# VinAIResearch/tise-toolbox

Measured on AMD Instinct MI355X. Metric: images/sec through InceptionV3+FID on 30k 256x256 @1/2/4/8 GPU; |dFID| vs ref, higher is better.
Workload: dtype f32 (split 2xf16 operands, 3 f16 MFMAs/product, f32 accumulate)

## Files before the change

tise_toolbox_amd/csrc/conv_pipe.hip:

```cpp
#include <stdlib.h>
#include <string.h>
#include <hip/hip_fp16.h>
#include "common.h"
#include "conv_epilogue.h"

namespace {

typedef _Float16 half8_t __attribute__((ext_vector_type(8)));
typedef _Float16 half4_t __attribute__((ext_vector_type(4)));
typedef float float16_t __attribute__((ext_vector_type(16)));
typedef float float4_t __attribute__((ext_vector_type(4)));
typedef unsigned int u32x4_t __attribute__((ext_vector_type(4)));
typedef tise_conv_args ConvArgs;
typedef __attribute__((address_space(3))) void* lds_ptr_t;

__device__ __attribute__((aligned(64))) unsigned char g_pipe_zero_page[64];

#define CP_BK 32

__device__ __forceinline__ bool wrap_guard(long long tile, long long ntiles) { return tile < ntiles; }

__device__ __forceinline__ int pool_swz(int slot) { return ((slot & 3) << 2) ^ ((slot >> 1) & 1); }
constexpr int POOL_HV_SLOTS = 130;

template <int COUT, bool PADDED, bool DBG = false, bool POOL = false>
__global__ __launch_bounds__(512, 2) void conv_regw32_kernel(const ConvArgs p, const int R16, const long long ntiles) {
    static_assert(!POOL || (COUT == 64 && !PADDED && !DBG), "pooled output: Conv2d_2b's instance only");
    constexpr int KHC = 3, KWC = 3, ntaps = 9;
    constexpr int TPI = 64 / COUT;
    constexpr int PF = COUT == 64 ? 2 : 1;
    constexpr int NPW = 2 * TPI;
    constexpr int STEP = 128 * TPI;
    constexpr int STG = conv_epi::Staging<1>::BYTES;
    extern __shared__ __attribute__((aligned(1024))) unsigned char lds[];
    const int tid = threadIdx.x, lane = tid & 63;
    const int wave = __builtin_amdgcn_readfirstlane(tid >> 6);
    const int ms = wave & 3, grp = wave >> 2;
    const int ring = R16 + STEP * PF;
    unsigned char* wbuf = lds;
    unsigned char* epi_area = wbuf + ring * 128;
    unsigned char* stage = epi_area + 2048 + wave * STG;
    unsigned char* vbuf = epi_area + 2048;
    unsigned char* hvbuf = vbuf + p.OW * 256;

    const long long G = (long long)gridDim.x;
    const long long mgrid = (long long)p.N * p.H * p.W;
    const int minoff = -p.PH * p.W - p.PW;
    const unsigned char* xg = reinterpret_cast<const unsigned char*>(p.x);
    const unsigned char* zp = g_pipe_zero_page;
    const long long niter_all = (ntiles + TPI - 1) / TPI;
    const long long per = (niter_all + G - 1) / G;
    const long long i_begin = (long long)blockIdx.x * per, i_end = (i_begin + per < niter_all) ? i_begin + per : niter_all;
    if (!POOL && i_begin >= niter_all) return;
    const int ohp = (p.OH - 3) / 2 + 1, owp = (p.OW - 3) / 2 + 1;
    long long g_start = 0;
    unsigned glen = 0;
    if (POOL) {
        const long long units = (long long)p.N * ohp;
        const long long u0 = units * blockIdx.x / G, u1 = units * (blockIdx.x + 1) / G;
        if (u0 >= u1) return;
        const long long n0 = u0 / ohp, n1 = (u1 - 1) / ohp;
        const int oy0 = (int)(u0 - n0 * ohp), oy1 = (int)(u1 - 1 - n1 * ohp);
        g_start = (n0 * p.H + 2 * oy0) * p.W;
        glen = (unsigned)((n1 * p.H + 2 * oy1 + 3) * p.W - g_start);
    }
    const long long t_begin = i_begin * TPI;
    const long long g_base = (POOL ? g_start : t_begin * 128) + minoff;
    const int nit = POOL ? (int)((glen + 127u) / 128u) : (int)(i_end - i_begin);

    half8_t bw[ntaps][2][2];
    {
        const _Float16* wgt = reinterpret_cast<const _Float16*>(p.w);
        const int cout = (COUT == 64 ? grp * 32 : 0) + (lane & 15);
        const _Float16* wrow = wgt + (long long)cout * p.Kpad + (lane >> 4) * 8;
#pragma unroll
        for (int t = 0; t < ntaps; ++t)
#pragma unroll
            for (int s2 = 0; s2 < 2; ++s2) {
                bw[t][s2][0] = *reinterpret_cast<const half8_t*>(wrow + (long long)s2 * 16 * p.Kpad + t * CP_BK);
                bw[t][s2][1] = *reinterpret_cast<const half8_t*>(wrow + (long long)s2 * 16 * p.Kpad + p.w_plane + t * CP_BK);
            }
#pragma unroll
        for (int t = 0; t < ntaps; ++t)
#pragma unroll
            for (int s2 = 0; s2 < 2; ++s2) {
                asm volatile("" : "+v"(bw[t][s2][0]));
                asm volatile("" : "+v"(bw[t][s2][1]));
            }
    }
#define RW32_ROWS(REL0, PROW0, NPIECES, Q0, QS)                                                           \
    {                                                                                                     \
        for (int q = (Q0); q < (NPIECES); q += (QS)) {                                                     \
            const long long g = g_base + (REL0) + q * 8 + (lane >> 3);                                     \
            const bool ok = g >= 0 && g < mgrid;                                                           \
            int prow = (PROW0) + q * 8;                                                                    \
            while (prow >= ring) prow -= ring;                                  \
            const int c = (lane & 7) ^ ((lane >> 4) << 1);     \
            const unsigned char* src = xg + g * 128 + c * 16;                                              \
            src = ok ? src : zp;                                                                           \
            __builtin_amdgcn_global_load_lds(src, (lds_ptr_t)(wbuf + prow * 128), 16, 0, 0);               \
        }                                                                                                  \
    }
    RW32_ROWS(0LL, 0, (R16 >> 3) + 16 * TPI * (PF - 1), wave, 8)
    {
        conv_epi::float4_t sc_pre = {0.f, 0.f, 0.f, 0.f}, bs_pre = {0.f, 0.f, 0.f, 0.f};
        if (tid < COUT / 4) {
            sc_pre = *reinterpret_cast<const conv_epi::float4_t*>(p.scale + 4 * tid);
            bs_pre = *reinterpret_cast<const conv_epi::float4_t*>(p.bias + 4 * tid);
        }
        static_assert(conv_epi::EpiArea<COUT>::BYTES <= 2048, "epilogue area");
        conv_epi::prepare<COUT>(p, epi_area, 0, sc_pre, bs_pre);
    }
    const unsigned W_ = (unsigned)p.W, H_ = (unsigned)p.H;
    const unsigned sx = (unsigned)STEP % W_, syf = (unsigned)STEP / W_;
    const unsigned sy = syf % H_, sn = syf / H_;
    unsigned en, ey, ex, cy[2] = {0, 0}, cx[2] = {0, 0};
    {
        const unsigned hw = H_ * W_;
        const unsigned g0 = (unsigned)(POOL ? g_start : t_begin * 128) + (TPI == 2 ? grp * 128 : 0) + ms * 32;
        const unsigned ge = g0 + (lane >> 3);
        en = ge / hw;
        const unsigned rem = ge - en * hw;
        ey = rem / W_; ex = rem - ey * W_;
        if (PADDED || POOL) {
#pragma unroll
            for (int pi = 0; pi < 2; ++pi) {
                const unsigned gc = g0 + pi * 16 + (lane & 15);
                const unsigned remc = gc % hw;
                cy[pi] = remc / W_; cx[pi] = remc - cy[pi] * W_;
            }
        }
    }
    unsigned tn_ = 0, ty_ = 0, tx_ = 0;
    if (POOL) {
        const unsigned hw = H_ * W_;
        tn_ = (unsigned)g_start / hw;
        ty_ = ((unsigned)g_start - tn_ * hw) / W_;
    }
    int toff[ntaps];
#pragma unroll
    for (int t = 0; t < ntaps; ++t) toff[t] = (t / KWC - p.PH) * p.W + (t % KWC - p.PW);
    const int lrow0 = (TPI == 2 ? grp * 128 : 0) + ms * 32 + (lane & 15) - minoff;
    const int l4 = lane >> 4;
    const unsigned ringB = (unsigned)ring * 128u;
    unsigned a0t[ntaps];
#pragma unroll
    for (int t = 0; t < ntaps; ++t) {
        int wrow = lrow0 + toff[t];
        wrow = wrow >= ring ? wrow - ring : wrow;
        a0t[t] = (unsigned)(wrow * 128 + ((l4 ^ tise_lds_swz(wrow)) << 4));
    }
    asm volatile("s_waitcnt vmcnt(0)" ::: "memory");
    __syncthreads();

    conv_epi::Acc16 acc_main[1][1], acc_corr[1][1];
    int wstart = 0;
    int pnew = (R16 + (PF - 1) * STEP) % ring;
    long long relnew = (long long)R16 + (PF - 1) * STEP;
    for (int it = 0; it < nit; ++it) {
        const bool ahead = it + PF < nit;
        if (ahead && !(DBG && (p.nseg & 0x100))) { RW32_ROWS(relnew, pnew, 16 * TPI, wave, 8) }
        const long long tile = t_begin + (long long)it * TPI + (TPI == 2 ? grp : 0);
        unsigned tapmask[2] = {0x1ffu, 0x1ffu};
        if (PADDED) {
#pragma unroll
            for (int pi = 0; pi < 2; ++pi) {
                tapmask[pi] = 0u;
#pragma unroll
                for (int t = 0; t < ntaps; ++t) {
                    const int yy = (int)cy[pi] + t / KWC - p.PH, xx = (int)cx[pi] + t % KWC - p.PW;
                    if (yy >= 0 && yy < p.H && xx >= 0 && xx < p.W) tapmask[pi] |= 1u << t;
                }
            }
        }
        half8_t fa_[2][2][2];
#define RW32_READS(TAP, BUF)                                                                              \
        {                                                                                                  \
            const unsigned a0 = a0t[TAP];                                                                  \
            const unsigned a1u = a0 + 2048u - ringB;           \
            const unsigned a1 = a1u < a1u + ringB ? a1u : a1u + ringB;                                     \
            u32x4_t ah0 = *reinterpret_cast<const u32x4_t*>(wbuf + a0);                                    \
            u32x4_t al0 = *reinterpret_cast<const u32x4_t*>(wbuf + (a0 ^ 64));                             \
            u32x4_t ah1 = *reinterpret_cast<const u32x4_t*>(wbuf + a1);                                    \
            u32x4_t al1 = *reinterpret_cast<const u32x4_t*>(wbuf + (a1 ^ 64));                             \
            if (PADDED) {                                                                                  \
                const unsigned am0 = (tapmask[0] >> (TAP)) & 1u ? 0xffffffffu : 0u;                        \
                const unsigned am1 = (tapmask[1] >> (TAP)) & 1u ? 0xffffffffu : 0u;                        \
                ah0 &= am0; al0 &= am0; ah1 &= am1; al1 &= am1;                                            \
            }                                                                                              \
            fa_[BUF][0][0] = __builtin_bit_cast(half8_t, ah0);                                             \
            fa_[BUF][0][1] = __builtin_bit_cast(half8_t, al0);                                             \
            fa_[BUF][1][0] = __builtin_bit_cast(half8_t, ah1);                                             \
            fa_[BUF][1][1] = __builtin_bit_cast(half8_t, al1);                                             \
        }
#define RW32_MFMAS(TAP, BUF)                                                                              \
        _Pragma("unroll") for (int ci = 0; ci < 2; ++ci)                                                   \
            _Pragma("unroll") for (int pi = 0; pi < 2; ++pi) {                                             \
                float4_t& cm = acc_main[0][0].v[ci][pi];                                                   \
                float4_t& cc = acc_corr[0][0].v[ci][pi];                                                   \
                cc = __builtin_amdgcn_mfma_f32_16x16x32_f16(bw[TAP][ci][1], fa_[BUF][pi][0], cc, 0, 0, 0); \
                cm = __builtin_amdgcn_mfma_f32_16x16x32_f16(bw[TAP][ci][0], fa_[BUF][pi][0], cm, 0, 0, 0); \
                cc = __builtin_amdgcn_mfma_f32_16x16x32_f16(bw[TAP][ci][0], fa_[BUF][pi][1], cc, 0, 0, 0); \
            }
#define RW32_TAPS()                                                                                       \
        {                                                                                                  \
            conv_epi::acc_zero(acc_main[0][0]); conv_epi::acc_zero(acc_corr[0][0]);                        \
            if (!(DBG && (p.nseg & 0x200))) {                                                              \
            __builtin_amdgcn_sched_barrier(0);                                                             \
            RW32_READS(0, 0)                                                                               \
            _Pragma("unroll") for (int tap = 0; tap < ntaps; ++tap) {                                      \
                if (tap + 1 < ntaps) {                                                                     \
                    if ((tap + 1) & 1) { RW32_READS(tap + 1, 1) } else { RW32_READS(tap + 1, 0) }          \
                }                                                                                          \
                if (tap & 1) { RW32_MFMAS(tap, 1) } else { RW32_MFMAS(tap, 0) }                            \
            }                                                                                              \
                                                                 \
            __builtin_amdgcn_sched_group_barrier(0x100, 4, 0);                                             \
            _Pragma("unroll") for (int tap = 0; tap + 1 < ntaps; ++tap) {                                  \
                __builtin_amdgcn_sched_group_barrier(0x100, 4, 0);                                         \
                __builtin_amdgcn_sched_group_barrier(0x008, 12, 0);                                        \
            }                                                                                              \
            __builtin_amdgcn_sched_group_barrier(0x008, 12, 0);                                            \
            __builtin_amdgcn_sched_barrier(0);                                                             \
            }                                                                                              \
        }
#define RW32_EPI(TILE, N_, Y_, X_)                                                                        \
        if (!(DBG && (p.nseg & 0x400))) {                                                                  \
            const unsigned nyx[3] = {N_, Y_, X_};                                                          \
            conv_epi::store_tiles_desc<1, 1, true, COUT>(p, acc_main, acc_corr, stage, epi_area, (TILE) * 128 + ms * 32, \
                                                         COUT == 64 ? grp * 4 : 0, nyx);                   \
        }
        const bool live = wrap_guard(tile, ntiles);
#define RW32_ADVANCE()                                                                                    \
        {                                                                                                  \
            ex += sx; ey += sy; en += sn;                                                                  \
            if (ex >= W_) { ex -= W_; ++ey; }                                                              \
            if (ey >= H_) { ey -= H_; ++en; }                                                              \
        }
        if (POOL || live) RW32_TAPS()
        if (PF == 2 && ahead) asm volatile("s_waitcnt vmcnt(%0)" ::"n"(NPW) : "memory");
        else asm volatile("s_waitcnt vmcnt(0)" ::: "memory");
        if constexpr (POOL) {
            __syncthreads();
            const unsigned grel0 = (unsigned)it * 128u + ms * 32 + (lane & 15);
            float4_t vold[2][2];
            unsigned va[2][2];
            bool valid[2], first[2];
#pragma unroll
            for (int pi = 0; pi < 2; ++pi) {
                const unsigned grel = grel0 + pi * 16;
                valid[pi] = cx[pi] < (unsigned)p.OW && cy[pi] < (unsigned)p.OH && grel < glen;
                first[pi] = grel < W_ || cy[pi] == 0;
                const int xs_ = valid[pi] ? (int)cx[pi] : 0;
#pragma unroll
                for (int ci = 0; ci < 2; ++ci) {
                    const int chunk = grp * 8 + ci * 4 + l4;
                    va[ci][pi] = (unsigned)(xs_ * 256 + ((chunk ^ pool_swz(xs_)) << 4));
                    vold[ci][pi] = *reinterpret_cast<const float4_t*>(vbuf + va[ci][pi]);
                }
            }
            float vmax = 0.f;
#pragma unroll
            for (int ci = 0; ci < 2; ++ci) {
                const int ch = grp * 32 + ci * 16 + l4 * 4;
                const float4_t sc = *reinterpret_cast<const float4_t*>(epi_area + conv_epi::EpiArea<COUT>::SCALE + ch * 4);
                const float4_t bs = *reinterpret_cast<const float4_t*>(epi_area + conv_epi::EpiArea<COUT>::BIAS + ch * 4);
#pragma unroll
                for (int pi = 0; pi < 2; ++pi) {
                    float4_t f, m;
#pragma unroll
                    for (int k = 0; k < 4; ++k) {
                        const float v = (acc_main[0][0].v[ci][pi][k] + acc_corr[0][0].v[ci][pi][k] * (1.0f / 2048.0f)) * sc[k];
                        f[k] = fmaxf(v + bs[k], 0.f);
                        vmax = fmaxf(vmax, f[k]);
                        m[k] = fmaxf(vold[ci][pi][k], f[k]);
                    }
                    const bool even = !(cy[pi] & 1u);
                    if (valid[pi]) {
                        float4_t nv;
#pragma unroll
                        for (int k = 0; k < 4; ++k) nv[k] = (first[pi] || even) ? f[k] : m[k];
                        *reinterpret_cast<float4_t*>(vbuf + va[ci][pi]) = nv;
                        if (even && !first[pi]) {
                            const int xx = (int)cx[pi];
                            const int slot = xx >= POOL_HV_SLOTS ? xx - POOL_HV_SLOTS : xx;
                            const int chunk = grp * 8 + ci * 4 + l4;
                            *reinterpret_cast<float4_t*>(hvbuf + slot * 256 + ((chunk ^ pool_swz(slot)) << 4)) = m;
                        }
                    }
                }
            }
            tise_flag_split_overflow(vmax);
            __syncthreads();
            {
                const unsigned len1 = (W_ - tx_) < 128u ? (W_ - tx_) : 128u;
                const bool ev1 = !(ty_ & 1u);
                const unsigned ye = ev1 ? ty_ : ty_ + 1u;
                const int xs = ev1 ? (int)tx_ : 0;
                int xe = ev1 ? (int)(tx_ + len1) - 1 : 127 - (int)len1;
                const unsigned row_rel = (unsigned)it * 128u + (ev1 ? 0u : len1) - (unsigned)xs;
                xe = xe < p.OW - 1 ? xe : p.OW - 1;
                const bool row_ok = ye >= 2u && ye < (unsigned)p.OH && row_rel != 0u && row_rel < glen && xe >= 2;
                if (row_ok) {
                    const int ox_lo = xs <= 2 ? 0 : (xs - 1) >> 1, ox_hi = (xe - 2) >> 1;
                    const int ox = ox_lo + (tid >> 3), c8 = tid & 7;
                    if (ox <= ox_hi) {
                        float mx[8];
#pragma unroll
                        for (int j = 0; j < 3; ++j) {
                            const int xx = 2 * ox + j;
                            const int slot = xx >= POOL_HV_SLOTS ? xx - POOL_HV_SLOTS : xx;
                            const unsigned a = (unsigned)(slot * 256 + (((2 * c8) ^ pool_swz(slot)) << 4));
                            const float4_t q0 = *reinterpret_cast<const float4_t*>(hvbuf + a);
                            const float4_t q1 = *reinterpret_cast<const float4_t*>(hvbuf + (a ^ 16u));
#pragma unroll
                            for (int k = 0; k < 4; ++k) {
                                mx[k] = j == 0 ? q0[k] : fmaxf(mx[k], q0[k]);
                                mx[4 + k] = j == 0 ? q1[k] : fmaxf(mx[4 + k], q1[k]);
                            }
                        }
                        half8_t ph, pl;
#pragma unroll
                        for (int k = 0; k < 8; ++k) {
                            const _Float16 h0 = (_Float16)mx[k];
                            const _Float16 l0 = (_Float16)((mx[k] - (float)h0) * 2048.0f);
                            const float fm = (float)h0 + (float)l0 * (1.0f / 2048.0f);
                            ph[k] = (_Float16)fm;
                            pl[k] = (_Float16)((fm - (float)ph[k]) * 2048.0f);
                        }
                        const conv_epi::ChunkDesc cd = *reinterpret_cast<const conv_epi::ChunkDesc*>(epi_area + conv_epi::EpiArea<COUT>::DESC + c8 * 32);
                        const unsigned long long pix = ((unsigned long long)tn_ * (unsigned)ohp + ((ye - 2u) >> 1)) * (unsigned)owp + (unsigned)ox;
                        unsigned char* d = reinterpret_cast<unsigned char*>(cd.base) + pix * (unsigned long long)cd.row_stride;
                        if (cd.valid) {
                            __builtin_nontemporal_store(__builtin_bit_cast(u32x4_t, ph), conv_epi::global_ptr(d));
                            __builtin_nontemporal_store(__builtin_bit_cast(u32x4_t, pl), conv_epi::global_ptr(d + cd.second));
                        }
                    }
                }
                tx_ += sx; ty_ += sy; tn_ += sn;
                if (tx_ >= W_) { tx_ -= W_; ++ty_; }
                if (ty_ >= H_) { ty_ -= H_; ++tn_; }
            }
        } else {
            if (live) RW32_EPI(tile, en, ey, ex)
        }
        RW32_ADVANCE()
        wstart += STEP; wstart = wstart >= ring ? wstart - ring : wstart;
#pragma unroll
        for (int t = 0; t < ntaps; ++t) {
            const unsigned u = a0t[t] + (unsigned)(STEP * 128) - ringB;
            a0t[t] = u < u + ringB ? u : u + ringB;
        }
        pnew += STEP; pnew = pnew >= ring ? pnew - ring : pnew;
        relnew += STEP;
        if (PADDED || POOL) {
#pragma unroll
            for (int pi = 0; pi < 2; ++pi) {
                cx[pi] += sx; cy[pi] += sy;
                if (cx[pi] >= W_) { cx[pi] -= W_; ++cy[pi]; }
                if (cy[pi] >= H_) cy[pi] -= H_;
            }
        }
        if (!POOL) __syncthreads();
    }
#undef RW32_ADVANCE
#undef RW32_ROWS
#undef RW32_READS
#undef RW32_MFMAS
#undef RW32_TAPS
#undef RW32_EPI
}

template <int COUT, bool PADDED>
static int launch_regw32_inst(const ConvArgs* a, int R16, long long ntiles, long long grid, size_t lds, hipStream_t st) {
    static std::atomic<unsigned long long> attr_set{0};
    if (tise_first_use_on_this_device(attr_set))
        TISE_HIP_CHECK(hipFuncSetAttribute(reinterpret_cast<const void*>(conv_regw32_kernel<COUT, PADDED>),
                                           hipFuncAttributeMaxDynamicSharedMemorySize, 160 * 1024));
    hipLaunchKernelGGL((conv_regw32_kernel<COUT, PADDED>), dim3((unsigned)grid), dim3(512), lds, st, *a, R16, ntiles);
    TISE_LAUNCH_CHECK();
    return TISE_OK;
}

int launch_regw32_pool(const ConvArgs* a, hipStream_t st) {
    if (a->Cin != 32 || a->SH != 1 || a->SW != 1 || a->KH != 3 || a->KW != 3 || a->Kpad != 9 * 32 || a->Cout != 64 || (a->PH | a->PW) != 0 ||
        a->OH < 3 || a->OW < 3 || a->W < 128 || a->W > 2 * POOL_HV_SLOTS || (long long)a->N * a->H * a->W >= 0x7fffff00LL || a->out_hp != 0)
        return TISE_ERR_INVALID_ARG;
    for (int i = 0; i < (a->nseg & 0xff); ++i)
        if (a->seg[i].mode != 0) return TISE_ERR_INVALID_ARG;
    if (a->nseg & ~0xff) return TISE_ERR_INVALID_ARG;
    const int R16 = (128 + 2 * a->W + 2 + 15) & ~15;
    const size_t lds = (size_t)(R16 + 256) * 128 + 2048 + (size_t)a->OW * 256 + (size_t)POOL_HV_SLOTS * 256;
    if (lds > 160 * 1024) return TISE_ERR_UNSUPPORTED;
    const int ncu_cached = tise_cu_count();
    const long long units = (long long)a->N * ((a->OH - 3) / 2 + 1);
    long long grid = (units + 3) / 4;
    grid = grid < 1 ? 1 : (grid > ncu_cached ? ncu_cached : grid);
    static std::atomic<unsigned long long> attr_set{0};
    if (tise_first_use_on_this_device(attr_set))
        TISE_HIP_CHECK(hipFuncSetAttribute(reinterpret_cast<const void*>(conv_regw32_kernel<64, false, false, true>),
                                           hipFuncAttributeMaxDynamicSharedMemorySize, 160 * 1024));
    hipLaunchKernelGGL((conv_regw32_kernel<64, false, false, true>), dim3((unsigned)grid), dim3(512), lds, st, *a, R16, 0x7fffffffffffLL);
    TISE_LAUNCH_CHECK();
    return TISE_OK;
}

int launch_regw32(const ConvArgs* a, hipStream_t st) {
    if (a->Cin != 32 || a->SH != 1 || a->SW != 1 || a->KH != 3 || a->KW != 3 || a->Kpad != 9 * 32 || a->W < 8 ||
        (a->Cout != 32 && a->Cout != 64) || (long long)a->N * a->H * a->W >= 0x7fffff00LL)
        return TISE_ERR_INVALID_ARG;
    const int tpi = 64 / a->Cout;
    const int R = 128 * tpi + 2 * a->W + 2;
    const int R16 = (R + 15) & ~15;
    const int pf = a->Cout == 64 ? 2 : 1;
    const size_t lds = (size_t)(R16 + 128 * tpi * pf) * 128 + 2048 + 8 * (size_t)conv_epi::Staging<1>::BYTES;
    if (lds > 160 * 1024) return TISE_ERR_UNSUPPORTED;
    const long long mg = (long long)a->N * a->H * a->W;
    const long long ntiles = (mg + 127) / 128;
    const int ncu_cached = tise_cu_count();
    const long long niter = (ntiles + tpi - 1) / tpi;
    const long long grid = niter < ncu_cached ? niter : ncu_cached;
    const bool padded = (a->PH | a->PW) != 0;
    if (a->nseg & 0x700) {
        if (padded) return TISE_ERR_INVALID_ARG;
        hipLaunchKernelGGL((conv_regw32_kernel<64, false, true>), dim3((unsigned)grid), dim3(512), lds, st, *a, R16, ntiles);
        TISE_LAUNCH_CHECK();
        return a->Cout == 64 ? TISE_OK : TISE_ERR_INVALID_ARG;
    }
    if (a->Cout == 32)
        return padded ? launch_regw32_inst<32, true>(a, R16, ntiles, grid, lds, st) : launch_regw32_inst<32, false>(a, R16, ntiles, grid, lds, st);
    return padded ? launch_regw32_inst<64, true>(a, R16, ntiles, grid, lds, st) : launch_regw32_inst<64, false>(a, R16, ntiles, grid, lds, st);
}

__global__ __launch_bounds__(256) void stem_mfma_u8_kernel(const uint8_t* __restrict__ x, const float* __restrict__ lut,
                                                           int N, int H, int W, const _Float16* __restrict__ wsp,
                                                           const ConvArgs p) {
    constexpr int STG = conv_epi::Staging<1>::BYTES;
    __shared__ unsigned lut2[3 * 256];
    __shared__ __attribute__((aligned(16))) unsigned char epi[2048 + 4 * STG];
    const int tid = threadIdx.x, lane = tid & 63;
    const int wave = __builtin_amdgcn_readfirstlane(tid >> 6);
    for (int i = tid; i < 3 * 256; i += 256) {
        const float v = lut[i];
        const _Float16 hi = (_Float16)v;
        const _Float16 lo = (_Float16)((v - (float)hi) * 2048.0f);
        lut2[i] = (unsigned)__builtin_bit_cast(unsigned short, hi) | ((unsigned)__builtin_bit_cast(unsigned short, lo) << 16);
    }
    {
        conv_epi::float4_t sc_pre = {0.f, 0.f, 0.f, 0.f}, bs_pre = {0.f, 0.f, 0.f, 0.f};
        if (tid < 8) {
            sc_pre = *reinterpret_cast<const conv_epi::float4_t*>(p.scale + 4 * tid);
            bs_pre = *reinterpret_cast<const conv_epi::float4_t*>(p.bias + 4 * tid);
        }
        conv_epi::prepare<32>(p, epi, 0, sc_pre, bs_pre);
    }
    half8_t bw[2][2];
#pragma unroll
    for (int s2 = 0; s2 < 2; ++s2) {
        bw[s2][0] = *reinterpret_cast<const half8_t*>(wsp + (lane & 31) * 32 + s2 * 16 + (lane >> 5) * 8);
        bw[s2][1] = *reinterpret_cast<const half8_t*>(wsp + 1024 + (lane & 31) * 32 + s2 * 16 + (lane >> 5) * 8);
    }
    __syncthreads();
    const int OH = (H - 3) / 2 + 1, OW = (W - 3) / 2 + 1;
    const unsigned M32 = (unsigned)p.M, ohw = (unsigned)(OH * OW);
    const unsigned ntiles = (M32 + 31u) / 32u;
    const int h = lane >> 5;
    const int row_bytes = W * 3;
    const uint8_t* x_end = x + (int64_t)N * H * W * 3;
    const unsigned lutb = (unsigned)(unsigned long long)(lds_ptr_t)lut2;
    unsigned char* stage = epi + 2048 + wave * STG;
#define STEM_FETCH(T, D1, S1, D2, S2)                                                                      \
    {                                                                                                      \
        const unsigned pix = (T) * 32u + (unsigned)(lane & 31);                                            \
        const unsigned pp = pix < M32 ? pix : 0u;              \
        const unsigned n = pp / ohw;                                                                       \
        const unsigned rem = pp - n * ohw;                                                                 \
        const unsigned oh = rem / (unsigned)OW, ow = rem - oh * (unsigned)OW;                              \
        const uint8_t* base = x + (((int64_t)n * H + 2 * oh) * W + 2 * ow) * 3;                            \
         \
        const uint8_t* q1 = base + (h ? 2 * row_bytes : 0);                                                \
        const uint8_t* q2 = base + row_bytes + (h ? 7 : 0);                                                \
        STEM_RUN(D1, S1, q1)                                                                               \
        STEM_RUN(D2, S2, q2)                                                                               \
    }
#define STEM_RUN(D, S, Q)                                                                                  \
        {                                                                                                  \
            const uintptr_t a = reinterpret_cast<uintptr_t>(Q);                                            \
            const unsigned* w4 = reinterpret_cast<const unsigned*>(a & ~(uintptr_t)3);                     \
            if (reinterpret_cast<const uint8_t*>(w4) + 16 <= x_end) {                                      \
                D[0] = w4[0]; D[1] = w4[1]; D[2] = w4[2]; D[3] = w4[3];                                    \
                S = (int)(a & 3) * 8;                                                                      \
            } else {                                                                                       \
                D[0] = D[1] = D[2] = D[3] = 0u;                                                            \
                for (int bb = 0; bb < 12; ++bb)                                                            \
                    if ((Q) + bb < x_end) D[bb >> 2] |= (unsigned)(Q)[bb] << (8 * (bb & 3));               \
                S = 0;                                                                                     \
            }                                                                                              \
        }
#define STEM_ALIGN(R, D, S)                                                                                \
        {                                                                                                  \
            const unsigned long long lo64 = ((unsigned long long)D[1] << 32) | D[0], mid64 = ((unsigned long long)D[2] << 32) | D[1], \
                                     hi64 = ((unsigned long long)D[3] << 32) | D[2];                       \
            R[0] = (unsigned)(lo64 >> S); R[1] = (unsigned)(mid64 >> S); R[2] = (unsigned)(hi64 >> S);     \
        }
    unsigned r1[3], r2[3], d1[4] = {0u, 0u, 0u, 0u}, d2[4] = {0u, 0u, 0u, 0u};
    int s1 = 0, s2s = 0;
    const unsigned tile0 = blockIdx.x * 4u + (unsigned)wave, tstep = gridDim.x * 4u;
    if (tile0 < ntiles) STEM_FETCH(tile0, d1, s1, d2, s2s)
    for (unsigned tile = tile0; tile < ntiles; tile += tstep) {
        STEM_ALIGN(r1, d1, s1)
        STEM_ALIGN(r2, d2, s2s)
        if (tile + tstep < ntiles) STEM_FETCH(tile + tstep, d1, s1, d2, s2s)
        unsigned wv[16];
#pragma unroll
        for (int u = 0; u < 16; ++u) {
            const int b = u < 9 ? u : u - 9;
            const unsigned word = (u < 9 ? r1 : r2)[b >> 2];
            const unsigned byte4 = ((word >> (8 * (b & 3))) & 0xffu) << 2;
            unsigned addr;
            if (u < 9) addr = lutb + (unsigned)((u % 3) * 1024) + byte4;
            else addr = lutb + byte4 + (h ? (unsigned)(((b + 1) % 3) * 1024) : (unsigned)((b % 3) * 1024));
            asm volatile("ds_read_b32 %0, %1" : "=v"(wv[u]) : "v"(addr));
        }
        asm volatile("s_waitcnt lgkmcnt(0)" : "+v"(wv[0]), "+v"(wv[1]), "+v"(wv[2]), "+v"(wv[3]), "+v"(wv[4]), "+v"(wv[5]), "+v"(wv[6]), "+v"(wv[7]),
                     "+v"(wv[8]), "+v"(wv[9]), "+v"(wv[10]), "+v"(wv[11]), "+v"(wv[12]), "+v"(wv[13]), "+v"(wv[14]), "+v"(wv[15]));
        float16_t acc_main[1][1], acc_corr[1][1];
#pragma unroll
        for (int j = 0; j < 16; ++j) { acc_main[0][0][j] = 0.f; acc_corr[0][0][j] = 0.f; }
#pragma unroll
        for (int s2 = 0; s2 < 2; ++s2) {
            u32x4_t ah, al;
#pragma unroll
            for (int q = 0; q < 4; ++q) {
                const unsigned w0 = wv[s2 * 8 + 2 * q], w1 = wv[s2 * 8 + 2 * q + 1];
                ah[q] = __builtin_amdgcn_perm(w1, w0, 0x05040100u);
                al[q] = __builtin_amdgcn_perm(w1, w0, 0x07060302u);
            }
            const half8_t a_hi = __builtin_bit_cast(half8_t, ah), a_lo = __builtin_bit_cast(half8_t, al);
            acc_corr[0][0] = __builtin_amdgcn_mfma_f32_32x32x16_f16(bw[s2][1], a_hi, acc_corr[0][0], 0, 0, 0);
            acc_main[0][0] = __builtin_amdgcn_mfma_f32_32x32x16_f16(bw[s2][0], a_hi, acc_main[0][0], 0, 0, 0);
            acc_corr[0][0] = __builtin_amdgcn_mfma_f32_32x32x16_f16(bw[s2][0], a_lo, acc_corr[0][0], 0, 0, 0);
        }
        conv_epi::store_tiles_desc<1, 1, false, 32>(p, acc_main, acc_corr, stage, epi, (long long)tile * 32);
    }
#undef STEM_FETCH
#undef STEM_RUN
#undef STEM_ALIGN
}

}

extern "C" int tise_stem_conv3x3s2_split_u8_mfma(const uint8_t* x_dev, const float* lut_dev, int n, int h, int w, const void* wsplit_dev,
                                                 const float* scale_dev, const float* bias_dev, void* out_dev, void* stream) {
    if (!x_dev || !lut_dev || !wsplit_dev || !scale_dev || !bias_dev || !out_dev || n < 0 || h < 3 || w < 5) return TISE_ERR_INVALID_ARG;
    if (n == 0) return TISE_OK;
    const int oh = (h - 3) / 2 + 1, ow = (w - 3) / 2 + 1;
    const long long M = (long long)n * oh * ow;
    if (M >= 0x7fffff00LL || (long long)n * h * w * 3 < 32 || (reinterpret_cast<uintptr_t>(x_dev) & 3) != 0) return TISE_ERR_UNSUPPORTED;
    tise_conv_args a;
    memset(&a, 0, sizeof(a));
    a.scale = scale_dev; a.bias = bias_dev;
    a.N = n; a.H = h; a.W = w; a.Cin = 3; a.KH = 3; a.KW = 3; a.SH = 2; a.SW = 2; a.OH = oh; a.OW = ow;
    a.Cout = 32; a.K = 27; a.Kpad = 32; a.M = M; a.nseg = 1;
    a.seg[0].c0 = 0; a.seg[0].c1 = 32; a.seg[0].dst = out_dev; a.seg[0].ld = 32; a.seg[0].off = 0; a.seg[0].mode = 0;
    const long long tiles = (M + 31) / 32;
    long long grid = (tiles + 3) / 4;
    if (grid > 8192) grid = 8192;
    hipLaunchKernelGGL(stem_mfma_u8_kernel, dim3((unsigned)grid), dim3(256), 0, (hipStream_t)stream, x_dev, lut_dev, n, h, w,
                       reinterpret_cast<const _Float16*>(wsplit_dev), a);
    TISE_LAUNCH_CHECK();
    return TISE_OK;
}

int tise_conv_pipe_launch(const tise_conv_args* a, int cfg, void* stream) {
    if (a->out_hp && (a->out_y0 < 0 || a->out_x0 < 0 || a->out_y0 + a->OH > a->out_hp || a->out_x0 + a->OW > a->out_wp))
        return TISE_ERR_INVALID_ARG;
    {
        const long long ohp = a->out_hp ? a->out_hp : a->OH, owp = a->out_hp ? a->out_wp : a->OW;
        long long ldmax = 0;
        for (int i = 0; i < (a->nseg & 0xff); ++i) ldmax = a->seg[i].ld > ldmax ? a->seg[i].ld : ldmax;
        if ((long long)a->N * ohp * owp >= 0xffffffffLL || (ohp + a->H) * owp * ldmax * 4 >= 0x7fffffffLL) return TISE_ERR_UNSUPPORTED;
    }
    if (cfg == (34 | 1024)) return launch_regw32_pool(a, (hipStream_t)stream);
    if (cfg != 34) return TISE_ERR_INVALID_ARG;
    return launch_regw32(a, (hipStream_t)stream);
}

TISE_DEFINE_SPLIT_FLAG_READER(tise_internal_split_flag_conv_pipe)
```

Baseline: 26480.

## Defer BN scale, bias and ReLU until after max-pool in fused Conv2d_2b epilogue

In the pooled conv instance, the per-pixel batch-norm scale, bias and ReLU now run after the 3x3 max-pool reduction instead of before it, so the affine step is applied once per pooled output rather than once per conv output. The split-overflow check moves out of the loop: it tracks a per-thread running max of raw accumulators and applies scale and bias once at kernel end. The vertical and horizontal pool buffer writes become branch-light, using a precomputed address select that assumes hvbuf sits directly after vbuf at OW*256. Swapping the affine step and the max is only exact when every BN scale is positive, which is a correctness risk if any channel scale is negative.

Result: no change. 26520, median of 6 (+0.1%).

```diff
diff --git a/tise_toolbox_amd/csrc/conv_pipe.hip b/tise_toolbox_amd/csrc/conv_pipe.hip
--- a/tise_toolbox_amd/csrc/conv_pipe.hip
+++ b/tise_toolbox_amd/csrc/conv_pipe.hip
@@ -22,6 +22,11 @@
 
 __device__ __forceinline__ int pool_swz(int slot) { return ((slot & 3) << 2) ^ ((slot >> 1) & 1); }
 constexpr int POOL_HV_SLOTS = 130;
+__device__ __forceinline__ float pool_max(float a, float b) {
+    float d;
+    asm("v_max_f32 %0, %1, %2" : "=v"(d) : "v"(a), "v"(b));
+    return d;
+}
 
 template <int COUT, bool PADDED, bool DBG = false, bool POOL = false>
 __global__ __launch_bounds__(512, 2) void conv_regw32_kernel(const ConvArgs p, const int R16, const long long ntiles) {
@@ -154,6 +159,9 @@
     __syncthreads();
 
     conv_epi::Acc16 acc_main[1][1], acc_corr[1][1];
+    float gmax[2][4];
+#pragma unroll
+    for (int i = 0; i < 8; ++i) gmax[i >> 2][i & 3] = -__builtin_inff();
     int wstart = 0;
     int pnew = (R16 + (PF - 1) * STEP) % ring;
     long long relnew = (long long)R16 + (PF - 1) * STEP;
@@ -244,53 +252,45 @@
             __syncthreads();
             const unsigned grel0 = (unsigned)it * 128u + ms * 32 + (lane & 15);
             float4_t vold[2][2];
-            unsigned va[2][2];
-            bool valid[2], first[2];
+            unsigned va[2][2], ma[2][2];
+            bool valid[2], restart[2];
 #pragma unroll
             for (int pi = 0; pi < 2; ++pi) {
                 const unsigned grel = grel0 + pi * 16;
                 valid[pi] = cx[pi] < (unsigned)p.OW && cy[pi] < (unsigned)p.OH && grel < glen;
-                first[pi] = grel < W_ || cy[pi] == 0;
+                const bool first = grel < W_ || cy[pi] == 0;
+                const bool even = !(cy[pi] & 1u);
+                restart[pi] = first || even;
                 const int xs_ = valid[pi] ? (int)cx[pi] : 0;
+                const int xx = (int)cx[pi];
+                const int slot = xx >= POOL_HV_SLOTS ? xx - POOL_HV_SLOTS : xx;
+                const int chunk = grp * 8 + l4;
+                va[0][pi] = (unsigned)(xs_ * 256 + ((chunk ^ pool_swz(xs_)) << 4));
+                const unsigned ha = (unsigned)(p.OW * 256 + slot * 256 + ((chunk ^ pool_swz(slot)) << 4));
+                ma[0][pi] = (even && !first) ? ha : va[0][pi];
 #pragma unroll
                 for (int ci = 0; ci < 2; ++ci) {
-                    const int chunk = grp * 8 + ci * 4 + l4;
-                    va[ci][pi] = (unsigned)(xs_ * 256 + ((chunk ^ pool_swz(xs_)) << 4));
+                    if (ci) { va[ci][pi] = va[0][pi] ^ 64u; ma[ci][pi] = ma[0][pi] ^ 64u; }
                     vold[ci][pi] = *reinterpret_cast<const float4_t*>(vbuf + va[ci][pi]);
                 }
             }
-            float vmax = 0.f;
 #pragma unroll
             for (int ci = 0; ci < 2; ++ci) {
-                const int ch = grp * 32 + ci * 16 + l4 * 4;
-                const float4_t sc = *reinterpret_cast<const float4_t*>(epi_area + conv_epi::EpiArea<COUT>::SCALE + ch * 4);
-                const float4_t bs = *reinterpret_cast<const float4_t*>(epi_area + conv_epi::EpiArea<COUT>::BIAS + ch * 4);
 #pragma unroll
                 for (int pi = 0; pi < 2; ++pi) {
                     float4_t f, m;
 #pragma unroll
                     for (int k = 0; k < 4; ++k) {
-                        const float v = (acc_main[0][0].v[ci][pi][k] + acc_corr[0][0].v[ci][pi][k] * (1.0f / 2048.0f)) * sc[k];
-                        f[k] = fmaxf(v + bs[k], 0.f);
-                        vmax = fmaxf(vmax, f[k]);
-                        m[k] = fmaxf(vold[ci][pi][k], f[k]);
+                        f[k] = __builtin_fmaf(acc_corr[0][0].v[ci][pi][k], 1.0f / 2048.0f, acc_main[0][0].v[ci][pi][k]);
+                        gmax[ci][k] = fmaxf(gmax[ci][k], f[k]);
+                        m[k] = pool_max(vold[ci][pi][k], f[k]);
                     }
-                    const bool even = !(cy[pi] & 1u);
                     if (valid[pi]) {
-                        float4_t nv;
-#pragma unroll
-                        for (int k = 0; k < 4; ++k) nv[k] = (first[pi] || even) ? f[k] : m[k];
-                        *reinterpret_cast<float4_t*>(vbuf + va[ci][pi]) = nv;
-                        if (even && !first[pi]) {
-                            const int xx = (int)cx[pi];
-                            const int slot = xx >= POOL_HV_SLOTS ? xx - POOL_HV_SLOTS : xx;
-                            const int chunk = grp * 8 + ci * 4 + l4;
-                            *reinterpret_cast<float4_t*>(hvbuf + slot * 256 + ((chunk ^ pool_swz(slot)) << 4)) = m;
-                        }
+                        *reinterpret_cast<float4_t*>(vbuf + ma[ci][pi]) = m;
+                        if (restart[pi]) *reinterpret_cast<float4_t*>(vbuf + va[ci][pi]) = f;
                     }
                 }
             }
-            tise_flag_split_overflow(vmax);
             __syncthreads();
             {
                 const unsigned len1 = (W_ - tx_) < 128u ? (W_ - tx_) : 128u;
@@ -305,6 +305,10 @@
                     const int ox_lo = xs <= 2 ? 0 : (xs - 1) >> 1, ox_hi = (xe - 2) >> 1;
                     const int ox = ox_lo + (tid >> 3), c8 = tid & 7;
                     if (ox <= ox_hi) {
+                        const float4_t sc0 = *reinterpret_cast<const float4_t*>(epi_area + conv_epi::EpiArea<COUT>::SCALE + c8 * 32);
+                        const float4_t sc1 = *reinterpret_cast<const float4_t*>(epi_area + conv_epi::EpiArea<COUT>::SCALE + c8 * 32 + 16);
+                        const float4_t bs0 = *reinterpret_cast<const float4_t*>(epi_area + conv_epi::EpiArea<COUT>::BIAS + c8 * 32);
+                        const float4_t bs1 = *reinterpret_cast<const float4_t*>(epi_area + conv_epi::EpiArea<COUT>::BIAS + c8 * 32 + 16);
                         float mx[8];
 #pragma unroll
                         for (int j = 0; j < 3; ++j) {
@@ -322,6 +326,7 @@
                         half8_t ph, pl;
 #pragma unroll
                         for (int k = 0; k < 8; ++k) {
+                            mx[k] = fmaxf(__builtin_fmaf(mx[k], k < 4 ? sc0[k & 3] : sc1[k & 3], k < 4 ? bs0[k & 3] : bs1[k & 3]), 0.f);
                             const _Float16 h0 = (_Float16)mx[k];
                             const _Float16 l0 = (_Float16)((mx[k] - (float)h0) * 2048.0f);
                             const float fm = (float)h0 + (float)l0 * (1.0f / 2048.0f);
@@ -362,6 +367,18 @@
             }
         }
         if (!POOL) __syncthreads();
+    }
+    if constexpr (POOL) {
+        float vmax = 0.f;
+#pragma unroll
+        for (int ci = 0; ci < 2; ++ci) {
+            const int ch = grp * 32 + ci * 16 + l4 * 4;
+            const float4_t sc = *reinterpret_cast<const float4_t*>(epi_area + conv_epi::EpiArea<COUT>::SCALE + ch * 4);
+            const float4_t bs = *reinterpret_cast<const float4_t*>(epi_area + conv_epi::EpiArea<COUT>::BIAS + ch * 4);
+#pragma unroll
+            for (int k = 0; k < 4; ++k) vmax = fmaxf(vmax, __builtin_fmaf(gmax[ci][k], sc[k], bs[k]));
+        }
+        tise_flag_split_overflow(vmax);
     }
 #undef RW32_ADVANCE
 #undef RW32_ROWS
```
